# xdspacelab/openvslam

Hardware: NVIDIA H100
Metric: frames/sec extract+match+local-BA @1920x960 4000kp (higher is better)
Workload: dtype u8 (extract, Hamming) + f64 (pose optimiser, local BA)

## Files before the change

openvslam_b200/csrc/optimize.cu:

```cuda
#include <algorithm>
#include <cfloat>
#include <cmath>
#include <cstdio>
#include <cstdlib>
#include <cstring>
#include <new>
#include <sched.h>
#include <time.h>
#include <vector>


#include "ba_math.cuh"
#include "ovs_common.h"

namespace {

using ovs::CameraD;

constexpr int kMaxReducedDimBig = 6000;
constexpr int kCholMaxDynSmem = 226 * 1024;
constexpr int kNB = 32;
constexpr int kCholThreads = 512;
constexpr int kCholCluster = 8;
constexpr int kPoseThreads = 256;
// ... 62 lines not shown
    int stopped;
    int spec_width;
    int round_live;
    int need_more;
    int pending_nbatch;
    int num_rounds, num_iterations, num_trials, batches, solver_trials;
    int round_iterations[8];
    double lambda_init[8];
    double last_chi2, last_lambda;
};

struct BaDev {
    CameraD cam;
    int K, L, M, nfree, n;
    const double* poses; const double* points;
    const double* poses_ring; const double* points_ring;
    const int* obs_kf; const int* obs_lm; const float2* obs_xy; const float* obs_xr; const float* inv_sigma_sq;
    const unsigned char* level;
    const int* free_idx;
    const int* lm_first;
    int use_huber; double delta;
};

__global__ void __launch_bounds__(128) k_ba_linearize(BaDev P, const LmCtl* __restrict__ ctl, double* __restrict__ Hpl, double* __restrict__ Cpp,
                                                       double* __restrict__ bpo, double* __restrict__ All, double* __restrict__ blo) {
    if (!ctl->active) return;
    __shared__ __align__(16) double sm[128 * 30];
    P.poses = P.poses_ring + (size_t)ctl->cur * 12 * P.K; P.points = P.points_ring + (size_t)ctl->cur * 3 * P.L;
    P.use_huber = ctl->use_huber;
    const int base = blockIdx.x * 128, t = threadIdx.x;
    const int i = base + t;
    const int nedge = min(128, P.M - base);
    const bool live = i < P.M && !P.level[i];
    int dim = 0, fi = -1;
    double e[3] = {0, 0, 0}, Jp[18], Jl[9], ww = 0;
#pragma unroll
    for (int k = 0; k < 18; ++k) Jp[k] = 0;
#pragma unroll
    for (int k = 0; k < 9; ++k) Jl[k] = 0;
    if (live) {
        const int kf = P.obs_kf[i], lm = P.obs_lm[i];
        fi = P.free_idx[kf];
        const float xr = P.obs_xr ? P.obs_xr[i] : -1.0f;
        const bool stereo = xr >= 0.0f;
        const float2 xy = P.obs_xy[i];
        const double obs[3] = {(double)xy.x, (double)xy.y, (double)xr};
        double pose[12], pw[3];
#pragma unroll
        for (int k = 0; k < 12; ++k) pose[k] = P.poses[12 * (size_t)kf + k];
#pragma unroll
        for (int k = 0; k < 3; ++k) pw[k] = P.points[3 * (size_t)lm + k];
        dim = ovs::edge_eval(P.cam, pose, pw, obs, stereo, e, Jp, Jl);
        const double w = (double)P.inv_sigma_sq[i];
        double chi = 0;
        for (int d = 0; d < dim; ++d) chi += w * e[d] * e[d];
        double rho0 = chi, rho1 = 1.0;
        if (P.use_huber) ovs::huber(chi, P.delta, &rho0, &rho1);
        ww = rho1 * w;
    }
    double* sW = sm; double* sbp = sm + 128 * 18; double* sA = sbp + 128 * 6;
    {
        double* A = sA + 6 * t;
        for (int a = 0; a < 3; ++a)
            for (int b = a; b < 3; ++b) {
                double h = 0;
                for (int d = 0; d < dim; ++d) h += Jl[3 * d + a] * ww * Jl[3 * d + b];
                A[ovs::sym3(a, b)] = h;
            }
        double* W = sW + 18 * t; double* bp = sbp + 6 * t;
        const bool fr = fi >= 0;
        for (int a = 0; a < 6; ++a) {
            double g = 0;
            for (int d = 0; d < dim; ++d) g -= Jp[6 * d + a] * ww * e[d];
            bp[a] = fr ? g : 0.0;
            for (int b = 0; b < 3; ++b) {
                double h = 0;
                for (int d = 0; d < dim; ++d) h += Jp[6 * d + a] * ww * Jl[3 * d + b];
                W[3 * a + b] = fr ? h : 0.0;
            }
        }
    }
    __syncthreads();
    {
        const double2* s2 = reinterpret_cast<const double2*>(sW); double2* g2 = reinterpret_cast<double2*>(Hpl + 18 * (size_t)base);
        for (int q = t; q < 9 * nedge; q += 128) g2[q] = s2[q];
        s2 = reinterpret_cast<const double2*>(sbp); g2 = reinterpret_cast<double2*>(bpo + 6 * (size_t)base);
        for (int q = t; q < 3 * nedge; q += 128) g2[q] = s2[q];
        s2 = reinterpret_cast<const double2*>(sA); g2 = reinterpret_cast<double2*>(All + 6 * (size_t)base);
        for (int q = t; q < 3 * nedge; q += 128) g2[q] = s2[q];
    }
    __syncthreads();
    double* sC = sm; double* sbl = sm + 128 * 21;
    {
        double* C = sC + 21 * t; double* bl = sbl + 3 * t;
        const bool fr = fi >= 0;
        for (int a = 0; a < 6; ++a)
            for (int b = a; b < 6; ++b) {
                double h = 0;
                for (int d = 0; d < dim; ++d) h += Jp[6 * d + a] * ww * Jp[6 * d + b];
                C[ovs::sym6(a, b)] = fr ? h : 0.0;
            }
        for (int a = 0; a < 3; ++a) {
            double g = 0;
            for (int d = 0; d < dim; ++d) g -= Jl[3 * d + a] * ww * e[d];
            bl[a] = g;
        }
    }
    __syncthreads();
    {
        const double2* s2 = reinterpret_cast<const double2*>(sC); double2* g2 = reinterpret_cast<double2*>(Cpp + 21 * (size_t)base);
        const int nd = 21 * nedge;
        for (int q = t; q < nd / 2; q += 128) g2[q] = s2[q];
        if ((nd & 1) && t == 0) Cpp[21 * (size_t)base + nd - 1] = sC[nd - 1];
        const int nb = 3 * nedge;
        for (int q = t; q < nb; q += 128) blo[3 * (size_t)base + q] = sbl[q];
    }
}

__global__ void __launch_bounds__(128) k_ba_landmark_accum(BaDev P, const LmCtl* __restrict__ ctl, const double* __restrict__ All, const double* __restrict__ blo,
                                                            double* __restrict__ Hll, double* __restrict__ bl, double* __restrict__ maxdiag) {
    if (!ctl->active) return;
    const int l = blockIdx.x * 128 + threadIdx.x;
    double md = 0;
    if (l < P.L) {
        double H[6] = {0, 0, 0, 0, 0, 0}, b[3] = {0, 0, 0};
        for (int p = P.lm_first[l]; p < P.lm_first[l + 1]; ++p) {
            if (P.level[p]) continue;
#pragma unroll
            for (int k = 0; k < 6; ++k) H[k] += All[6 * (size_t)p + k];
#pragma unroll
            for (int k = 0; k < 3; ++k) b[k] += blo[3 * (size_t)p + k];
        }
#pragma unroll
        for (int k = 0; k < 6; ++k) Hll[6 * (size_t)l + k] = H[k];
#pragma unroll
        for (int k = 0; k < 3; ++k) bl[3 * (size_t)l + k] = b[k];
        md = fmax(fabs(H[0]), fmax(fabs(H[3]), fabs(H[5])));
    }
#pragma unroll
    for (int o = 16; o > 0; o >>= 1) md = fmax(md, __shfl_xor_sync(0xffffffffu, md, o));
    if ((threadIdx.x & 31) == 0 && md > 0) atomic_max_pos(maxdiag, md);
}

__global__ void __launch_bounds__(128) k_ba_pose_accum_chunk(BaDev P, const LmCtl* __restrict__ ctl, const int* __restrict__ nchunks,
                                                              const int4* __restrict__ pair_rec, const int4* __restrict__ chunks,
                                                              const double* __restrict__ Cpp, const double* __restrict__ bpo,
                                                              double* __restrict__ ppart) {
    __shared__ double red[27][4];
    if (!ctl->active || (int)blockIdx.x >= *nchunks) return;
    const int4 ch = chunks[blockIdx.x];
    const int e = ch.y + threadIdx.x;
    double acc[27];
#pragma unroll
    for (int k = 0; k < 27; ++k) acc[k] = 0;
    if (e < ch.z) {
        const int4 rec = pair_rec[e];
        const int o = rec.x;
        if (!rec.w) {
#pragma unroll
            for (int k = 0; k < 21; ++k) acc[k] = Cpp[21 * (size_t)o + k];
#pragma unroll
            for (int k = 0; k < 6; ++k) acc[21 + k] = bpo[6 * (size_t)o + k];
        }
    }
    const int lane = threadIdx.x & 31, wid = threadIdx.x >> 5;
#pragma unroll
    for (int k = 0; k < 27; ++k) {
        const double v = warp_sum(acc[k]);
        if (lane == 0) red[k][wid] = v;
    }
    __syncthreads();
    if (threadIdx.x < 27)
        ppart[27 * (size_t)blockIdx.x + threadIdx.x] = red[threadIdx.x][0] + red[threadIdx.x][1] + red[threadIdx.x][2] + red[threadIdx.x][3];
}

__global__ void k_ba_pose_final_plan(LmCtl* ctl, int nfree, const int* __restrict__ kf_chunk_begin, const double* __restrict__ ppart,
                                     double* __restrict__ Hpp, double* __restrict__ bp, double* maxdiag, int* fail,
                                     const volatile int* stop_word, volatile int* mirror);

__device__ __forceinline__ void dmma_m8n8k4(double& d0, double& d1, double a, double b) {
    asm volatile("mma.sync.aligned.m8n8k4.row.col.f64.f64.f64.f64 {%0, %1}, {%2}, {%3}, {%0, %1};\n" : "+d"(d0), "+d"(d1) : "d"(a), "d"(b));
}

constexpr int kSGY = 76, kSGW = 84;
__global__ void __launch_bounds__(128, 4) k_ba_schur_chunk(BaDev P, const LmCtl* __restrict__ ctl, const int* __restrict__ nchunks,
                                                         const int4* __restrict__ pair_rec, const int4* __restrict__ chunks,
                                                         const int2* __restrict__ pair_ab, const double* __restrict__ Hll,
                                                         const double* __restrict__ Hpl, const double* __restrict__ bl,
                                                         double* __restrict__ spart, size_t spart_stride) {
    __shared__ double s_y[4 * 8 * kSGY];
    __shared__ double s_w[4 * 8 * kSGW];
    double* sYw = s_y + (threadIdx.x >> 5) * 8 * kSGY;
    double* sWw = s_w + (threadIdx.x >> 5) * 8 * kSGW;
    static_assert(4 * 8 * kSGY >= kSpec * 4 * 64, "reduction buffer must fit in the Y region");
    const int nbatch = ctl->nbatch;
    if (nbatch == 0 || (int)blockIdx.x >= *nchunks) return;
// ... 757 lines not shown
                ovs::pose_oplus(pose, u, out);
            } else {
#pragma unroll
                for (int j = 0; j < 12; ++j) out[j] = pose[j];
            }
            double* cand_poses = poses_ring + (size_t)buf[bt] * 12 * P.K;
#pragma unroll
            for (int j = 0; j < 12; ++j) cand_poses[12 * (size_t)k + j] = out[j];
            }
        }
    }
#pragma unroll
    for (int bt = 0; bt < kSpec; ++bt) {
        if (bt < nbatch) {
            const double tot = block_sum(sc[bt], sm);
            if (threadIdx.x == 0) partial_scale[(size_t)bt * gridDim.x + blockIdx.x] = tot;
        }
    }
}

__global__ void __launch_bounds__(128) k_ba_errors(BaDev P, const LmCtl* __restrict__ ctl, int at_current,
                                                    double* __restrict__ err, double* __restrict__ partial_chi) {
    __shared__ double sm[36];
    int slot;
    if (at_current) {
        if (!ctl->active) return;
        slot = ctl->cur;
    } else {
        if ((int)blockIdx.y >= ctl->nbatch) return;
        slot = ctl->buf[blockIdx.y];
    }
    P.use_huber = ctl->use_huber;
    P.poses = P.poses_ring + (size_t)slot * 12 * P.K;
    P.points = P.points_ring + (size_t)slot * 3 * P.L;
    err += (size_t)blockIdx.y * 3 * P.M; partial_chi += (size_t)blockIdx.y * gridDim.x;
    const int i = blockIdx.x * 128 + threadIdx.x;
    double c = 0;
    if (i < P.M && !P.level[i]) {
        const int kf = P.obs_kf[i];
        const float xr = P.obs_xr ? P.obs_xr[i] : -1.0f;
        const bool stereo = xr >= 0.0f;
        const float2 xy = P.obs_xy[i];
        const double obs[3] = {(double)xy.x, (double)xy.y, (double)xr};
        double pose[12], pw[3], e[3] = {0, 0, 0};
#pragma unroll
        for (int k = 0; k < 12; ++k) pose[k] = P.poses[12 * (size_t)kf + k];
        const size_t pi = P.obs_lm ? (size_t)P.obs_lm[i] : (size_t)i;
#pragma unroll
        for (int k = 0; k < 3; ++k) pw[k] = P.points[3 * pi + k];
        ovs::edge_eval(P.cam, pose, pw, obs, stereo, e, nullptr, nullptr);
        err[3 * (size_t)i] = e[0]; err[3 * (size_t)i + 1] = e[1]; err[3 * (size_t)i + 2] = stereo ? e[2] : 0.0;
        const double w = (double)P.inv_sigma_sq[i];
        double chi = w * (e[0] * e[0] + e[1] * e[1]);
        if (stereo) chi += w * e[2] * e[2];
        c = chi;
        if (P.use_huber) { double r1; ovs::huber(chi, P.delta, &c, &r1); }
    }
    const double tot = block_sum(c, sm);
    if (threadIdx.x == 0) partial_chi[blockIdx.x] = tot;
}

__device__ __forceinline__ void mirror_state(const LmCtl& c, volatile int* mirror) {
    if (!mirror) return;
    mirror[0] = c.nbatch; mirror[1] = c.active; mirror[3] = c.need_more; mirror[4] = c.it;
}

__global__ void __launch_bounds__(kSpec * 256) k_ba_reduce(LmCtl* ctl, int mode, const double* __restrict__ partial_chi, int nchi,
                                                           const double* __restrict__ partial_scale, int nscale, int* fail,
                                                           const volatile int* stop_word, int batch_index, int* exec_log, volatile int* mirror,
                                                           int halt_if_undecided, int next_width_cap) {
    __shared__ double sm[kSpec][2][8];
    const int nb = mode == 0 ? (ctl->active ? 1 : 0) : ctl->nbatch;
    if (nb == 0) {
        if (threadIdx.x == 0 && mode == 1 && exec_log && batch_index >= 0) exec_log[batch_index] = 0;
        return;
    }
    const int t = threadIdx.x >> 8, tl = threadIdx.x & 255, lane = tl & 31, w = tl >> 5;
    double a = 0, b = 0;
    if (t < nb) {
        const double* pc = partial_chi + (size_t)t * nchi;
        for (int i = tl; i < nchi; i += 256) a += pc[i];
        if (mode == 1) {
// ... 488 lines not shown
            int ws = wsum[lane];
#pragma unroll
            for (int o = 1; o < 32; o <<= 1) { const int u = __shfl_up_sync(0xffffffffu, ws, o); if (lane >= o) ws += u; }
            wsum[lane] = ws;
        }
        __syncthreads();
        const int excl = carry + (wid ? wsum[wid - 1] : 0) + v - c;
        if (i < count) chunk_begin[i] = excl;
        __syncthreads();
        if (tid == 1023) carry = excl + c;
        __syncthreads();
    }
    if (tid == 0) { chunk_begin[count] = carry; *total = carry; }
}

__global__ void __launch_bounds__(128) k_ba_chunk_fill(const int* __restrict__ ids, int count, const int* __restrict__ seg_begin,
                                                        const int* __restrict__ seg_end, const int* __restrict__ chunk_begin, int4* __restrict__ chunks) {
    const int i = blockIdx.x * 128 + threadIdx.x;
    if (i >= count) return;
    const int id = ids ? ids[i] : i;
    const int e1 = seg_end[id];
    int c = chunk_begin[i];
    for (int e0 = seg_begin[id]; e0 < e1; e0 += 128, ++c) chunks[c] = make_int4(i, e0, min(e0 + 128, e1), 0);
}

struct PoseOptArgs {
    CameraD cam;
    int n;
    const double* pts_w; const float2* obs_xy; const float* obs_xr; const float* inv_sigma_sq;
    double* pose;
    unsigned char* outlier;
    int num_trials, num_each_iter;
    double delta, chi2_2d, chi2_3d;
    double* stats;
};

__device__ bool solve6(const double* Hs , double lambda, const double* b, double* x) {
    double Lm[6][6];
    for (int i = 0; i < 6; ++i)
        for (int j = 0; j <= i; ++j) {
            double s = Hs[ovs::sym6(j, i)] + (i == j ? lambda : 0.0);
            for (int k = 0; k < j; ++k) s -= Lm[i][k] * Lm[j][k];
            if (i == j) {
                if (!(s > 0.0) || !isfinite(s)) return false;
                Lm[i][i] = sqrt(s);
            } else Lm[i][j] = s / Lm[j][j];
// ... 212 lines not shown
        const double e0 = err[3 * (size_t)i], e1 = err[3 * (size_t)i + 1], e2 = err[3 * (size_t)i + 2];
        fc[0] += w * (e0 * e0 + e1 * e1) + (stereo ? w * e2 * e2 : 0.0);
    }
    reduce_all(fc, 1);
    if (gtid == 0) {
        A.stats[0] = total_iters; A.stats[1] = total_trials; A.stats[2] = rounds; A.stats[3] = s_sys[0]; A.stats[4] = n - num_bad;
    }
    if (gtid < 12) A.pose[gtid] = s_pose[gtid];
}

}

struct ovs_ba_plan;
extern "C" void ovs_optimizer_destroy(ovs_optimizer* h);
struct ovs_optimizer {
    int device = 0;
    ovs_ba_plan* plan = nullptr;
    cudaStream_t stream = nullptr;
    cudaEvent_t ev[2]{};
    std::vector<cudaEvent_t> solver_ev;
    cudaGraphExec_t gx_iter = nullptr;
    int spec_width = kSpec;
    int spec_width2 = 0;
    int use_graphs = 0;
    int lm_host_sync = -1;
    bool pending = false;
    uint8_t* d_arena = nullptr; size_t d_cap = 0;
    uint8_t* h_arena = nullptr; size_t h_cap = 0;
    uint8_t* d_work = nullptr; size_t w_cap = 0;
    int* h_mirror = nullptr;
    int* d_mirror = nullptr;
    int chol_cluster = kCholCluster;
};

namespace {

struct Arena {
    uint8_t* base; size_t off, cap;
    template <typename T> T* take(size_t n) {
        off = (off + 255) / 256 * 256;
        T* p = reinterpret_cast<T*>(base + off);
        off += n * sizeof(T);
        return p;
    }
};

int ensure_arenas(ovs_optimizer* h, size_t dbytes, size_t hbytes) {
// ... 78 lines not shown
        stats->final_chi2 = hstats[3];
        for (int r = 0; r < 8 && r < stats->num_rounds; ++r) stats->lambda_init[r] = hstats[5 + r];
        float ms = 0; cudaEventElapsedTime(&ms, h->ev[0], h->ev[1]);
        stats->device_us = ms * 1000.f;
    }
    return OVS_OK;
}

struct ovs_ba_plan {
    bool valid = false;
    BaDev P{};
    int K = 0, L = 0, M = 0, nfree = 0, n = 0, npairs = 0, nb_obs = 0, nb_upd = 0;
    long long npair_entries = 0;
    size_t chol_smem = 0;
    int chol_dbuf = 0, chol_big = 0;
    double* hposes = nullptr; double* hpoints = nullptr; uint8_t* hout = nullptr;
    LmCtl* hctl = nullptr; int* hexec = nullptr; int exec_cap = 0;
    double *dposes_in = nullptr, *dpoints_in = nullptr;
    double *dposes_ring = nullptr, *dpoints_ring = nullptr;
    uint8_t* dlevel = nullptr; double* derr = nullptr;
    uint8_t* dout = nullptr;
    LmCtl* dctl = nullptr; int* dexec = nullptr;
    size_t spart_stride = 0, S_stride = 0, invL_stride = 0;
    double *dHpl = nullptr, *dCpp = nullptr, *dbpo = nullptr, *dAll = nullptr, *dblo = nullptr;
    double *dHll = nullptr, *dbl = nullptr, *dHpp = nullptr, *dbp = nullptr;
    double *dS = nullptr, *dbS = nullptr, *dx = nullptr, *dinvL = nullptr;
    int4* d_pair_rec = nullptr; int *dsegb = nullptr, *dsege = nullptr; int2* dpab = nullptr; int* ddiag = nullptr;
    int4 *dchunks = nullptr, *ddchunks = nullptr; int *dpair_chunk_begin = nullptr, *dkf_chunk_begin = nullptr;
    int* dnchunks = nullptr;
    double *dspart = nullptr, *dppart = nullptr; int max_chunks = 0, max_dchunks = 0;
    double *dpchi = nullptr, *dpscale = nullptr; int* dfail = nullptr; double* dmaxdiag = nullptr; long long* dclk = nullptr;
    int cur = 0;
};

namespace {

struct BaInputs {
    const double* poses; const uint8_t* fixed; const double* points; const int32_t* obs_kf; const int32_t* obs_lm;
    const float* obs_xy; const float* obs_x_right; const float* inv_sigma_sq;
};

int ensure_work(ovs_optimizer* h, size_t bytes) {
    if (bytes > h->w_cap) {
        cudaFree(h->d_work); h->d_work = nullptr; h->w_cap = 0;
        bytes += bytes / 4;
        OVS_CUDA_CHECK(cudaMalloc(&h->d_work, bytes));
        h->w_cap = bytes;
    }
    return OVS_OK;
}

int prepare_impl(ovs_optimizer* h, const ovs_camera* cam, int setup_is_mono, int K, int L, int M, const BaInputs& in, bool on_device) {
    OVS_REQUIRE(h && cam && K > 0 && L > 0 && M > 0, OVS_ERR_INVALID_ARG, "bad argument");
// ... 5 lines not shown
    cudaStream_t st = h->stream;
    if (h->pending) { OVS_CUDA_CHECK(ovs::sync_stream(st)); h->pending = false; }

    const size_t sM = (size_t)M, sL = (size_t)L, sK = (size_t)K;
    const int nb_obs = (M + 127) / 128, nb_upd = (L + K + 127) / 128;
    const int exec_cap = 1024;
    double* hposes; double* hpoints; int *hkf, *hlm; float *hxy, *hxr, *hw; uint8_t* hfixed; uint8_t* hout; long long* hcounts;
    double* dposes_in; double* dpoints_in; int *dkf, *dlm; float *dxy, *dxr, *dw; uint8_t* dfixed;
    int *dfree, *dlmf, *dpoff; long long* dcounts;
    size_t in_bytes = 0;
    auto carve1 = [&](Arena& H, Arena& D) {
        hposes = H.take<double>(12 * sK); hpoints = H.take<double>(3 * sL);
        hkf = H.take<int>(sM); hlm = H.take<int>(sM); hxy = H.take<float>(2 * sM); hxr = H.take<float>(sM); hw = H.take<float>(sM);
        hfixed = H.take<uint8_t>(sK);
        in_bytes = H.off;
        hout = H.take<uint8_t>(sM); pl.hctl = H.take<LmCtl>(1); pl.hexec = H.take<int>(exec_cap); hcounts = H.take<long long>(8);
        dposes_in = D.take<double>(12 * sK); dpoints_in = D.take<double>(3 * sL);
        dkf = D.take<int>(sM); dlm = D.take<int>(sM); dxy = D.take<float>(2 * sM); dxr = D.take<float>(sM); dw = D.take<float>(sM);
        dfixed = D.take<uint8_t>(sK);
        dfree = D.take<int>(sK); dlmf = D.take<int>(sL + 1); dpoff = D.take<int>(sL + 1); dcounts = D.take<long long>(8);
        pl.dout = D.take<uint8_t>(sM); pl.dctl = D.take<LmCtl>(1); pl.dexec = D.take<int>(exec_cap);
        pl.dposes_ring = D.take<double>((kSpec + 1) * 12 * sK); pl.dpoints_ring = D.take<double>((kSpec + 1) * 3 * sL);
        pl.dlevel = D.take<uint8_t>(sM); pl.derr = D.take<double>(kSpec * 3 * sM);
        pl.dHpl = D.take<double>(18 * sM); pl.dCpp = D.take<double>(21 * sM); pl.dbpo = D.take<double>(6 * sM);
        pl.dAll = D.take<double>(6 * sM); pl.dblo = D.take<double>(3 * sM);
        pl.dHll = D.take<double>(6 * sL); pl.dbl = D.take<double>(3 * sL);
        pl.dpchi = D.take<double>(kSpec * (size_t)nb_obs); pl.dpscale = D.take<double>(kSpec * (size_t)nb_upd);
        pl.dfail = D.take<int>(kSpec); pl.dmaxdiag = D.take<double>(2); pl.dclk = D.take<long long>(192); pl.dnchunks = D.take<int>(2);
    };
    {
        Arena H0{nullptr, 0, 0}, D0{nullptr, 0, 0};
        carve1(H0, D0);
        const int rc = ensure_arenas(h, D0.off + 256, H0.off + 256);
        if (rc != OVS_OK) return rc;
    }
    Arena H{h->h_arena, 0, h->h_cap}, D{h->d_arena, 0, h->d_cap};
    carve1(H, D);
    pl.exec_cap = exec_cap;
    h->pending = true;
    if (!on_device) {
        memcpy(hposes, in.poses, 96 * sK); memcpy(hpoints, in.points, 24 * sL);
        memcpy(hkf, in.obs_kf, 4 * sM); memcpy(hlm, in.obs_lm, 4 * sM); memcpy(hxy, in.obs_xy, 8 * sM); memcpy(hw, in.inv_sigma_sq, 4 * sM);
        if (in.obs_x_right) memcpy(hxr, in.obs_x_right, 4 * sM); else for (size_t i = 0; i < sM; ++i) hxr[i] = -1.0f;
        memcpy(hfixed, in.fixed, sK);
        OVS_CUDA_CHECK(cudaMemcpyAsync(h->d_arena, h->h_arena, in_bytes, cudaMemcpyHostToDevice, st));
    } else {
        const cudaMemcpyKind dd = cudaMemcpyDeviceToDevice;
// ... 16 lines not shown
    OVS_LAUNCH_CHECK();
    OVS_CUDA_CHECK(cudaMemcpyAsync(hcounts, dcounts, 5 * sizeof(long long), cudaMemcpyDeviceToHost, st));
    OVS_CUDA_CHECK(ovs::sync_stream(st));
    if (hcounts[4] != 0x7fffffffffffffffll) {
        const long long i = hcounts[4] >> 2;
        const int code = (int)(hcounts[4] & 3);
        h->pending = false;
        if (code == 2) { ovs::set_error("observations must be grouped by landmark (obs_lm non-decreasing; first violation at observation %lld)", i); return OVS_ERR_INVALID_ARG; }
        if (!on_device) ovs::set_error("observation %lld references keyframe %d / landmark %d out of range", i, in.obs_kf[i], in.obs_lm[i]);
        else ovs::set_error("observation %lld references a keyframe / landmark out of range", i);
        return OVS_ERR_INVALID_ARG;
    }
    const int nfree = (int)hcounts[0];
    const long long npair_entries = hcounts[1], nfree_edges = hcounts[2];
    const int n = 6 * nfree;
    OVS_REQUIRE(nfree >= 1, OVS_ERR_INVALID_ARG, "no free keyframe");
    OVS_REQUIRE(n <= kMaxReducedDimBig, OVS_ERR_UNSUPPORTED, "more than %d free keyframes", kMaxReducedDimBig / 6);
    OVS_REQUIRE(npair_entries < (1ll << 30), OVS_ERR_UNSUPPORTED, "too many co-observations");
    const int npairs = nfree * (nfree + 1) / 2;

    const size_t sE = (size_t)std::max<long long>(npair_entries, 1);
    const size_t max_chunks = sE / 128 + (size_t)npairs + 8;
    const size_t max_dchunks = (size_t)nfree_edges / 128 + (size_t)nfree + 8;
    unsigned *dkeys, *dkeys2; unsigned long long *dvals, *dvals2; int4* dprec; int* dsort;
    auto carve2 = [&](Arena& W) {
        pl.dpab = W.take<int2>(npairs); pl.ddiag = W.take<int>(nfree);
        pl.dHpp = W.take<double>(21 * (size_t)nfree); pl.dbp = W.take<double>(6 * (size_t)nfree);
        pl.S_stride = ((size_t)(n + 1) * n + 31) / 32 * 32; pl.invL_stride = (size_t)((n + kNB - 1) / kNB) * kNB * kNB;
        pl.dS = W.take<double>(kSpec * pl.S_stride); pl.dbS = pl.dS + (size_t)n * n; pl.dx = W.take<double>(kSpec * (size_t)n);
        pl.dinvL = W.take<double>(kSpec * pl.invL_stride);
        dkeys = W.take<unsigned>(sE); dkeys2 = W.take<unsigned>(sE);
        dvals = W.take<unsigned long long>(sE); dvals2 = W.take<unsigned long long>(sE); dprec = W.take<int4>(sE);
        dsort = W.take<int>(sort_scratch_ints((long long)sE));
        pl.dsegb = W.take<int>(npairs); pl.dsege = W.take<int>(npairs);
        pl.dchunks = W.take<int4>(max_chunks); pl.ddchunks = W.take<int4>(max_dchunks);
        pl.dpair_chunk_begin = W.take<int>(npairs + 1); pl.dkf_chunk_begin = W.take<int>(nfree + 1);
        pl.spart_stride = 42 * max_chunks;
        pl.dspart = W.take<double>(kSpec * pl.spart_stride); pl.dppart = W.take<double>(27 * max_dchunks);
    };
    {
        Arena W0{nullptr, 0, 0};
        carve2(W0);
        const int rc = ensure_work(h, W0.off + 256);
        if (rc != OVS_OK) return rc;
    }
    Arena W{h->d_work, 0, h->w_cap};
    carve2(W);
    pl.max_chunks = (int)max_chunks; pl.max_dchunks = (int)max_dchunks;
    OVS_CUDA_CHECK(cudaMemsetAsync(pl.dsegb, 0, 4 * (size_t)npairs, st));
    OVS_CUDA_CHECK(cudaMemsetAsync(pl.dsege, 0, 4 * (size_t)npairs, st));
    OVS_CUDA_CHECK(cudaMemsetAsync(pl.dS, 0, 8 * kSpec * pl.S_stride, st));

    BaDev& P = pl.P;
    P.cam = to_cam(cam); P.K = K; P.L = L; P.M = M; P.nfree = nfree; P.n = n;
    P.poses = dposes_in; P.points = dpoints_in; P.poses_ring = pl.dposes_ring; P.points_ring = pl.dpoints_ring;
    P.obs_kf = dkf; P.obs_lm = dlm; P.obs_xy = (const float2*)dxy; P.obs_xr = dxr; P.inv_sigma_sq = dw;
    P.level = pl.dlevel; P.free_idx = dfree; P.lm_first = dlmf;
    const float chi_sq_2D = 5.99146f, chi_sq_3D = 7.81473f;
    P.use_huber = 1; P.delta = (double)(setup_is_mono ? sqrtf(chi_sq_2D) : sqrtf(chi_sq_3D));

    k_ba_pair_table<<<nfree, 128, 0, st>>>(nfree, pl.dpab, pl.ddiag);
    OVS_LAUNCH_CHECK();
    pl.d_pair_rec = dprec;
    if (npair_entries > 0) {
        k_ba_emit_pairs<<<(L + 127) / 128, 128, 0, st>>>(P, dpoff, dkeys, dvals);
        OVS_LAUNCH_CHECK();
        int end_bit = 1;
        while ((1 << end_bit) < npairs) ++end_bit;
        unsigned* ksorted = nullptr; unsigned long long* vsorted = nullptr;
        const int src = sort_pairs(st, dkeys, dkeys2, dvals, dvals2, (int)npair_entries, end_bit, dsort, &ksorted, &vsorted);
        if (src != OVS_OK) return src;
        k_ba_segments<<<((int)npair_entries + 255) / 256, 256, 0, st>>>(ksorted, (int)npair_entries, pl.dsegb, pl.dsege);
        OVS_LAUNCH_CHECK();
        k_ba_pair_records<<<((int)npair_entries + 255) / 256, 256, 0, st>>>(vsorted, (int)npair_entries, dlm, dprec);
        OVS_LAUNCH_CHECK();
    }
    k_ba_chunk_scan<<<1, 1024, 0, st>>>(nullptr, npairs, pl.dsegb, pl.dsege, pl.dpair_chunk_begin, pl.dnchunks);
    OVS_LAUNCH_CHECK();
    k_ba_chunk_fill<<<(npairs + 127) / 128, 128, 0, st>>>(nullptr, npairs, pl.dsegb, pl.dsege, pl.dpair_chunk_begin, pl.dchunks);
    OVS_LAUNCH_CHECK();
    k_ba_chunk_scan<<<1, 1024, 0, st>>>(pl.ddiag, nfree, pl.dsegb, pl.dsege, pl.dkf_chunk_begin, pl.dnchunks + 1);
    OVS_LAUNCH_CHECK();
    k_ba_chunk_fill<<<(nfree + 127) / 128, 128, 0, st>>>(pl.ddiag, nfree, pl.dsegb, pl.dsege, pl.dkf_chunk_begin, pl.ddchunks);
    OVS_LAUNCH_CHECK();

    pl.K = K; pl.L = L; pl.M = M; pl.nfree = nfree; pl.n = n; pl.npairs = npairs; pl.nb_obs = nb_obs; pl.nb_upd = nb_upd;
    pl.npair_entries = npair_entries;
    {
        const size_t fixed = chol_fixed_doubles(n), panel = chol_panel_doubles(n), back = chol_back_doubles(n) - 32 * 33;
        const size_t one = (fixed + std::max(panel, back)) * sizeof(double);
        const size_t two = (fixed + std::max(panel, back + chol_back_doubles(n))) * sizeof(double);
        pl.chol_big = one > (size_t)kCholMaxDynSmem ? 1 : 0;
        pl.chol_dbuf = two <= (size_t)kCholMaxDynSmem ? 1 : 0;
        pl.chol_smem = pl.chol_big ? 0 : (pl.chol_dbuf ? two : one);
    }
    pl.hposes = hposes; pl.hpoints = hpoints; pl.hout = hout;
    pl.dposes_in = dposes_in; pl.dpoints_in = dpoints_in;
    pl.cur = 0;
    pl.valid = true;
    return OVS_OK;
}

}

extern "C" int ovs_local_ba_prepare(ovs_optimizer* h, const ovs_camera* cam, int setup_is_mono, int K, const double* poses,
                                    const uint8_t* fixed, int L, const double* points, int M, const int32_t* obs_kf,
                                    const int32_t* obs_lm, const float* obs_xy, const float* obs_x_right, const float* inv_sigma_sq) {
// ... 118 lines not shown
            OVS_CUDA_CHECK(cudaLaunchKernelEx(&cfg, k_ba_cholesky_solve, (const LmCtl*)ctl, pl.dS, pl.S_stride, n, pl.dx, pl.dinvL, pl.invL_stride, pl.dfail, pl.dclk, pl.chol_dbuf));
            ovs::count_launch();
        } else {
            for (int kb = 0; kb < n; kb += kNB) {
                const int nb = std::min(kNB, n - kb), rem = n - kb - nb, prow = rem + 1;
                k_chol_big_diag<<<dim3(1, kSpec), 64, 0, st>>>(ctl, pl.dS, pl.S_stride, n, kb, nb, pl.dinvL, pl.invL_stride, pl.dfail);
                OVS_LAUNCH_CHECK();
                k_chol_big_panel<<<dim3((prow + 127) / 128, kSpec), 128, 0, st>>>(ctl, pl.dS, pl.S_stride, n, kb, nb, pl.dinvL, pl.invL_stride);
                OVS_LAUNCH_CHECK();
                if (rem > 0) {
                    int tiles = 0;
                    for (int mi = 0; mi < (prow + 15) / 16; ++mi) tiles += std::min((rem + 31) / 32, (16 * mi + 15) / 32 + 1);
                    k_chol_big_trailing<<<dim3((tiles + 3) / 4, kSpec), 128, 0, st>>>(ctl, pl.dS, pl.S_stride, n, kb, nb);
                    OVS_LAUNCH_CHECK();
                }
            }
            const size_t bsm = (size_t)(((n + 31) / 32) * 32 + 32 * 33 + 32) * sizeof(double);
            k_chol_big_backsolve<<<kSpec, 512, bsm, st>>>(ctl, pl.dS, pl.S_stride, n, pl.dinvL, pl.invL_stride, pl.dx, pl.dfail);
            OVS_LAUNCH_CHECK();
        }
        if (ev) OVS_CUDA_CHECK(cudaEventRecord(h->solver_ev[4 * slot + 3], st));
        k_ba_update<<<nb_upd, 128, 0, st>>>(P, ctl, pl.dHpl, pl.dHll, pl.dbl, pl.dbp, pl.dx, pl.dposes_ring, pl.dpoints_ring, pl.dpscale, pl.dfail);
        OVS_LAUNCH_CHECK();
        k_ba_errors<<<dim3(nb_obs, kSpec), 128, 0, st>>>(P, ctl, 0, pl.derr, pl.dpchi);
        OVS_LAUNCH_CHECK();
        k_ba_reduce<<<1, kSpec * 256, 0, st>>>(ctl, 1, pl.dpchi, nb_obs, pl.dpscale, nb_upd, pl.dfail, stop_word, ev ? slot : -1, pl.dexec, mirror,
                                               halt_if_undecided ? 1 : 0, next_width_cap);
        OVS_LAUNCH_CHECK();
        if (!in_graph) ++solver_slots;
        return OVS_OK;
    };

    auto iteration_head = [&](bool in_graph, bool halt_if_undecided) -> int {
        k_ba_linearize<<<nb_obs, 128, 0, st>>>(P, ctl, pl.dHpl, pl.dCpp, pl.dbpo, pl.dAll, pl.dblo);
        OVS_LAUNCH_CHECK();
        k_ba_landmark_accum<<<(L + 127) / 128, 128, 0, st>>>(P, ctl, pl.dAll, pl.dblo, pl.dHll, pl.dbl, pl.dmaxdiag);
        OVS_LAUNCH_CHECK();
        k_ba_pose_accum_chunk<<<pl.max_dchunks, 128, 0, st>>>(P, ctl, pl.dnchunks + 1, pl.d_pair_rec, pl.ddchunks, pl.dCpp, pl.dbpo, pl.dppart);
        OVS_LAUNCH_CHECK();
        k_ba_pose_final_plan<<<1, 1024, 0, st>>>(ctl, nfree, pl.dkf_chunk_begin, pl.dppart, pl.dHpp, pl.dbp, pl.dmaxdiag, pl.dfail, stop_word, mirror);
        OVS_LAUNCH_CHECK();
        if (sw2 > 0 && halt_if_undecided) {
            const int rc = trial_batch(in_graph, false, sw2);
            if (rc != OVS_OK) return rc;
        }
        return trial_batch(in_graph, halt_if_undecided, 0);
    };

    auto finish_iteration = [&]() -> int {
        for (;;) {
            int rc = wait_device();
            if (rc != OVS_OK) return rc;
            if (hm[0] == 0) return OVS_OK;
            rc = trial_batch(false, false, 0);
            if (rc != OVS_OK) return rc;
        }
    };

    auto lm_optimize = [&](int iterations, int use_huber) -> int {
        k_lm_round_begin<<<1, 1, 0, st>>>(ctl, iterations, use_huber, stop_word, pl.dmaxdiag, mirror);
        OVS_LAUNCH_CHECK();
// ... 115 lines not shown
    return run_impl(h, 2, 1, num_first_iter, num_second_iter, force_stop_flag, stats);
}

extern "C" int ovs_global_ba_host(ovs_optimizer* h, const ovs_camera* cam, int setup_is_mono, int K, double* poses, const uint8_t* fixed,
                                  int L, double* points, int M, const int32_t* obs_kf, const int32_t* obs_lm, const float* obs_xy,
                                  const float* obs_x_right, const float* inv_sigma_sq, int num_iter, int use_huber_kernel,
                                  const volatile uint8_t* force_stop_flag, ovs_ba_stats* stats) {
    OVS_REQUIRE(h && cam && K > 0 && L >= 0 && M >= 0 && num_iter >= 0, OVS_ERR_INVALID_ARG, "bad argument");
    OVS_REQUIRE(poses && fixed && (L == 0 || points) && (M == 0 || (obs_kf && obs_lm && obs_xy && inv_sigma_sq)), OVS_ERR_INVALID_ARG, "null argument");
    if (stats) memset(stats, 0, sizeof(*stats));
    if (force_stop_flag && *force_stop_flag) return OVS_OK;
    if (M == 0 || L == 0) return OVS_OK;
    int rc = ovs_local_ba_prepare(h, cam, setup_is_mono, K, poses, fixed, L, points, M, obs_kf, obs_lm, obs_xy, obs_x_right, inv_sigma_sq);
    if (rc != OVS_OK) return rc;
    rc = run_impl(h, 1, use_huber_kernel ? 1 : 0, num_iter, 0, force_stop_flag, stats);
    if (rc != OVS_OK) return rc;
    return ovs_local_ba_fetch(h, poses, points, nullptr);
}

extern "C" int ovs_optimizer_cluster_width(const ovs_optimizer* h) { return h ? h->chol_cluster : 0; }

extern "C" int ovs_optimizer_set_cluster_width(ovs_optimizer* h, int width) {
    OVS_REQUIRE(h && (width == 1 || width == 2 || width == 4 || width == 8), OVS_ERR_INVALID_ARG, "cluster width must be 1, 2, 4 or 8");
    h->chol_cluster = width;
    return OVS_OK;
}

extern "C" int ovs_optimizer_set_speculation(ovs_optimizer* h, int width) {
    OVS_REQUIRE(h && width >= 1 && width <= kSpec, OVS_ERR_INVALID_ARG, "speculation width must be 1..%d", kSpec);
    h->spec_width = width;
    return OVS_OK;
}

extern "C" int ovs_optimizer_set_second_batch(ovs_optimizer* h, int width) {
    OVS_REQUIRE(h && width >= 0 && width <= kSpec, OVS_ERR_INVALID_ARG, "second-batch width must be 0..%d", kSpec);
    h->spec_width2 = width;
    return OVS_OK;
}

extern "C" int ovs_optimizer_set_graphs(ovs_optimizer* h, int enable) {
    OVS_REQUIRE(h, OVS_ERR_INVALID_ARG, "null handle");
    h->use_graphs = enable ? 1 : 0;
    return OVS_OK;
}

extern "C" int ovs_optimizer_set_host_sync(ovs_optimizer* h, int mode) {
// ... 138 lines not shown
```

Measured before the change: 387.1.

## Fuse pose accumulation into linearize, batch speculative error eval, enable graphs

Result: faster. 397.3, median of 6 (+2.6%).

```diff
diff --git a/openvslam_b200/csrc/optimize.cu b/openvslam_b200/csrc/optimize.cu
--- a/openvslam_b200/csrc/optimize.cu
+++ b/openvslam_b200/csrc/optimize.cu
@@ -108,99 +108,127 @@
     int use_huber; double delta;
 };
 
-__global__ void __launch_bounds__(128) k_ba_linearize(BaDev P, const LmCtl* __restrict__ ctl, double* __restrict__ Hpl, double* __restrict__ Cpp,
-                                                       double* __restrict__ bpo, double* __restrict__ All, double* __restrict__ blo) {
+__device__ __forceinline__ int ba_edge_linearize(const BaDev& P, int i, int lm, const double* pose, double* e, double* Jp, double* Jl, double& ww) {
+    const float xr = P.obs_xr ? P.obs_xr[i] : -1.0f;
+    const bool stereo = xr >= 0.0f;
+    const float2 xy = P.obs_xy[i];
+    const double obs[3] = {(double)xy.x, (double)xy.y, (double)xr};
+    double pw[3];
+#pragma unroll
+    for (int k = 0; k < 3; ++k) pw[k] = P.points[3 * (size_t)lm + k];
+    const int dim = ovs::edge_eval(P.cam, pose, pw, obs, stereo, e, Jp, Jl);
+    const double w = (double)P.inv_sigma_sq[i];
+    double chi = 0;
+    for (int d = 0; d < dim; ++d) chi += w * e[d] * e[d];
+    double rho0 = chi, rho1 = 1.0;
+    if (P.use_huber) ovs::huber(chi, P.delta, &rho0, &rho1);
+    ww = rho1 * w;
+    return dim;
+}
+__device__ __forceinline__ void ba_store_landmark_blocks(int i, int dim, const double* e, const double* Jl, double ww,
+                                                         double* __restrict__ All, double* __restrict__ blo) {
+    double A[6];
+#pragma unroll
+    for (int a = 0; a < 3; ++a)
+#pragma unroll
+        for (int b = a; b < 3; ++b) {
+            double h = 0;
+            for (int d = 0; d < dim; ++d) h += Jl[3 * d + a] * ww * Jl[3 * d + b];
+            A[ovs::sym3(a, b)] = h;
+        }
+    double2* A2 = reinterpret_cast<double2*>(All + 6 * (size_t)i);
+#pragma unroll
+    for (int k = 0; k < 3; ++k) A2[k] = make_double2(A[2 * k], A[2 * k + 1]);
+#pragma unroll
+    for (int a = 0; a < 3; ++a) {
+        double g = 0;
+        for (int d = 0; d < dim; ++d) g -= Jl[3 * d + a] * ww * e[d];
+        blo[3 * (size_t)i + a] = g;
+    }
+}
+
+__global__ void __launch_bounds__(128) k_ba_linearize(BaDev P, const LmCtl* __restrict__ ctl, const int* __restrict__ nchunks,
+                                                       const int4* __restrict__ pair_rec, const int4* __restrict__ chunks, int dchunk_cap,
+                                                       const int* __restrict__ fixed_edges, int nfixed, double* __restrict__ Hpl,
+                                                       double* __restrict__ All, double* __restrict__ blo, double* __restrict__ ppart) {
+    __shared__ double spose[12];
+    __shared__ double red[27][4];
     if (!ctl->active) return;
-    __shared__ __align__(16) double sm[128 * 30];
     P.poses = P.poses_ring + (size_t)ctl->cur * 12 * P.K; P.points = P.points_ring + (size_t)ctl->cur * 3 * P.L;
     P.use_huber = ctl->use_huber;
-    const int base = blockIdx.x * 128, t = threadIdx.x;
-    const int i = base + t;
-    const int nedge = min(128, P.M - base);
-    const bool live = i < P.M && !P.level[i];
-    int dim = 0, fi = -1;
+    const int t = threadIdx.x;
+    int dim = 0;
     double e[3] = {0, 0, 0}, Jp[18], Jl[9], ww = 0;
 #pragma unroll
     for (int k = 0; k < 18; ++k) Jp[k] = 0;
 #pragma unroll
     for (int k = 0; k < 9; ++k) Jl[k] = 0;
+    if ((int)blockIdx.x >= dchunk_cap) {
+        const int j = ((int)blockIdx.x - dchunk_cap) * 128 + t;
+        if (j >= nfixed) return;
+        const int i = fixed_edges[j];
+        if (!P.level[i]) {
+            const int kf = P.obs_kf[i];
+            double pose[12];
+#pragma unroll
+            for (int k = 0; k < 12; ++k) pose[k] = P.poses[12 * (size_t)kf + k];
+            dim = ba_edge_linearize(P, i, P.obs_lm[i], pose, e, Jp, Jl, ww);
+        }
+        ba_store_landmark_blocks(i, dim, e, Jl, ww, All, blo);
+        return;
+    }
+    if ((int)blockIdx.x >= *nchunks) return;
+    const int4 ch = chunks[blockIdx.x];
+    if (t < 12) spose[t] = P.poses[12 * (size_t)P.obs_kf[pair_rec[ch.y].x] + t];
+    const int r = ch.y + t;
+    const bool has = r < ch.z;
+    int4 rec = make_int4(0, 0, 0, 1);
+    if (has) rec = pair_rec[r];
+    const int i = rec.x;
+    const bool live = has && !P.level[i];
+    __syncthreads();
     if (live) {
-        const int kf = P.obs_kf[i], lm = P.obs_lm[i];
-        fi = P.free_idx[kf];
-        const float xr = P.obs_xr ? P.obs_xr[i] : -1.0f;
-        const bool stereo = xr >= 0.0f;
-        const float2 xy = P.obs_xy[i];
-        const double obs[3] = {(double)xy.x, (double)xy.y, (double)xr};
-        double pose[12], pw[3];
-#pragma unroll
-        for (int k = 0; k < 12; ++k) pose[k] = P.poses[12 * (size_t)kf + k];
-#pragma unroll
-        for (int k = 0; k < 3; ++k) pw[k] = P.points[3 * (size_t)lm + k];
-        dim = ovs::edge_eval(P.cam, pose, pw, obs, stereo, e, Jp, Jl);
-        const double w = (double)P.inv_sigma_sq[i];
-        double chi = 0;
-        for (int d = 0; d < dim; ++d) chi += w * e[d] * e[d];
-        double rho0 = chi, rho1 = 1.0;
-        if (P.use_huber) ovs::huber(chi, P.delta, &rho0, &rho1);
-        ww = rho1 * w;
-    }
-    double* sW = sm; double* sbp = sm + 128 * 18; double* sA = sbp + 128 * 6;
-    {
-        double* A = sA + 6 * t;
-        for (int a = 0; a < 3; ++a)
-            for (int b = a; b < 3; ++b) {
-                double h = 0;
-                for (int d = 0; d < dim; ++d) h += Jl[3 * d + a] * ww * Jl[3 * d + b];
-                A[ovs::sym3(a, b)] = h;
-            }
-        double* W = sW + 18 * t; double* bp = sbp + 6 * t;
-        const bool fr = fi >= 0;
-        for (int a = 0; a < 6; ++a) {
-            double g = 0;
-            for (int d = 0; d < dim; ++d) g -= Jp[6 * d + a] * ww * e[d];
-            bp[a] = fr ? g : 0.0;
+        double pose[12];
+#pragma unroll
+        for (int k = 0; k < 12; ++k) pose[k] = spose[k];
+        dim = ba_edge_linearize(P, i, rec.z, pose, e, Jp, Jl, ww);
+    }
+    if (has) {
+        double W[18];
+#pragma unroll
+        for (int a = 0; a < 6; ++a)
+#pragma unroll
             for (int b = 0; b < 3; ++b) {
                 double h = 0;
                 for (int d = 0; d < dim; ++d) h += Jp[6 * d + a] * ww * Jl[3 * d + b];
-                W[3 * a + b] = fr ? h : 0.0;
-            }
-        }
+                W[3 * a + b] = h;
+            }
+        double2* W2 = reinterpret_cast<double2*>(Hpl + 18 * (size_t)i);
+#pragma unroll
+        for (int k = 0; k < 9; ++k) W2[k] = make_double2(W[2 * k], W[2 * k + 1]);
+        ba_store_landmark_blocks(i, dim, e, Jl, ww, All, blo);
+    }
+    const bool add = has && !rec.w;
+    const int lane = t & 31, wid = t >> 5;
+#pragma unroll
+    for (int a = 0; a < 6; ++a)
+#pragma unroll
+        for (int b = a; b < 6; ++b) {
+            double h = 0;
+            for (int d = 0; d < dim; ++d) h += Jp[6 * d + a] * ww * Jp[6 * d + b];
+            const double v = warp_sum(add ? h : 0.0);
+            if (lane == 0) red[ovs::sym6(a, b)][wid] = v;
+        }
+#pragma unroll
+    for (int a = 0; a < 6; ++a) {
+        double g = 0;
+        for (int d = 0; d < dim; ++d) g -= Jp[6 * d + a] * ww * e[d];
+        const double v = warp_sum(add ? g : 0.0);
+        if (lane == 0) red[21 + a][wid] = v;
     }
     __syncthreads();
-    {
-        const double2* s2 = reinterpret_cast<const double2*>(sW); double2* g2 = reinterpret_cast<double2*>(Hpl + 18 * (size_t)base);
-        for (int q = t; q < 9 * nedge; q += 128) g2[q] = s2[q];
-        s2 = reinterpret_cast<const double2*>(sbp); g2 = reinterpret_cast<double2*>(bpo + 6 * (size_t)base);
-        for (int q = t; q < 3 * nedge; q += 128) g2[q] = s2[q];
-        s2 = reinterpret_cast<const double2*>(sA); g2 = reinterpret_cast<double2*>(All + 6 * (size_t)base);
-        for (int q = t; q < 3 * nedge; q += 128) g2[q] = s2[q];
-    }
-    __syncthreads();
-    double* sC = sm; double* sbl = sm + 128 * 21;
-    {
-        double* C = sC + 21 * t; double* bl = sbl + 3 * t;
-        const bool fr = fi >= 0;
-        for (int a = 0; a < 6; ++a)
-            for (int b = a; b < 6; ++b) {
-                double h = 0;
-                for (int d = 0; d < dim; ++d) h += Jp[6 * d + a] * ww * Jp[6 * d + b];
-                C[ovs::sym6(a, b)] = fr ? h : 0.0;
-            }
-        for (int a = 0; a < 3; ++a) {
-            double g = 0;
-            for (int d = 0; d < dim; ++d) g -= Jl[3 * d + a] * ww * e[d];
-            bl[a] = g;
-        }
-    }
-    __syncthreads();
-    {
-        const double2* s2 = reinterpret_cast<const double2*>(sC); double2* g2 = reinterpret_cast<double2*>(Cpp + 21 * (size_t)base);
-        const int nd = 21 * nedge;
-        for (int q = t; q < nd / 2; q += 128) g2[q] = s2[q];
-        if ((nd & 1) && t == 0) Cpp[21 * (size_t)base + nd - 1] = sC[nd - 1];
-        const int nb = 3 * nedge;
-        for (int q = t; q < nb; q += 128) blo[3 * (size_t)base + q] = sbl[q];
-    }
+    if (t < 27)
+        ppart[27 * (size_t)blockIdx.x + t] = red[t][0] + red[t][1] + red[t][2] + red[t][3];
 }
 
 __global__ void __launch_bounds__(128) k_ba_landmark_accum(BaDev P, const LmCtl* __restrict__ ctl, const double* __restrict__ All, const double* __restrict__ blo,
@@ -226,38 +254,6 @@
 #pragma unroll
     for (int o = 16; o > 0; o >>= 1) md = fmax(md, __shfl_xor_sync(0xffffffffu, md, o));
     if ((threadIdx.x & 31) == 0 && md > 0) atomic_max_pos(maxdiag, md);
-}
-
-__global__ void __launch_bounds__(128) k_ba_pose_accum_chunk(BaDev P, const LmCtl* __restrict__ ctl, const int* __restrict__ nchunks,
-                                                              const int4* __restrict__ pair_rec, const int4* __restrict__ chunks,
-                                                              const double* __restrict__ Cpp, const double* __restrict__ bpo,
-                                                              double* __restrict__ ppart) {
-    __shared__ double red[27][4];
-    if (!ctl->active || (int)blockIdx.x >= *nchunks) return;
-    const int4 ch = chunks[blockIdx.x];
-    const int e = ch.y + threadIdx.x;
-    double acc[27];
-#pragma unroll
-    for (int k = 0; k < 27; ++k) acc[k] = 0;
-    if (e < ch.z) {
-        const int4 rec = pair_rec[e];
-        const int o = rec.x;
-        if (!rec.w) {
-#pragma unroll
-            for (int k = 0; k < 21; ++k) acc[k] = Cpp[21 * (size_t)o + k];
-#pragma unroll
-            for (int k = 0; k < 6; ++k) acc[21 + k] = bpo[6 * (size_t)o + k];
-        }
-    }
-    const int lane = threadIdx.x & 31, wid = threadIdx.x >> 5;
-#pragma unroll
-    for (int k = 0; k < 27; ++k) {
-        const double v = warp_sum(acc[k]);
-        if (lane == 0) red[k][wid] = v;
-    }
-    __syncthreads();
-    if (threadIdx.x < 27)
-        ppart[27 * (size_t)blockIdx.x + threadIdx.x] = red[threadIdx.x][0] + red[threadIdx.x][1] + red[threadIdx.x][2] + red[threadIdx.x][3];
 }
 
 __global__ void k_ba_pose_final_plan(LmCtl* ctl, int nfree, const int* __restrict__ kf_chunk_begin, const double* __restrict__ ppart,
@@ -1061,42 +1057,56 @@
 __global__ void __launch_bounds__(128) k_ba_errors(BaDev P, const LmCtl* __restrict__ ctl, int at_current,
                                                     double* __restrict__ err, double* __restrict__ partial_chi) {
     __shared__ double sm[36];
-    int slot;
+    int nb, slot[kSpec];
     if (at_current) {
         if (!ctl->active) return;
-        slot = ctl->cur;
+        nb = 1; slot[0] = ctl->cur;
     } else {
-        if ((int)blockIdx.y >= ctl->nbatch) return;
-        slot = ctl->buf[blockIdx.y];
+        nb = ctl->nbatch;
+        if (nb == 0) return;
+#pragma unroll
+        for (int bt = 0; bt < kSpec; ++bt) slot[bt] = ctl->buf[bt];
     }
     P.use_huber = ctl->use_huber;
-    P.poses = P.poses_ring + (size_t)slot * 12 * P.K;
-    P.points = P.points_ring + (size_t)slot * 3 * P.L;
-    err += (size_t)blockIdx.y * 3 * P.M; partial_chi += (size_t)blockIdx.y * gridDim.x;
     const int i = blockIdx.x * 128 + threadIdx.x;
-    double c = 0;
+    double c[kSpec];
+#pragma unroll
+    for (int bt = 0; bt < kSpec; ++bt) c[bt] = 0;
     if (i < P.M && !P.level[i]) {
         const int kf = P.obs_kf[i];
         const float xr = P.obs_xr ? P.obs_xr[i] : -1.0f;
         const bool stereo = xr >= 0.0f;
         const float2 xy = P.obs_xy[i];
         const double obs[3] = {(double)xy.x, (double)xy.y, (double)xr};
-        double pose[12], pw[3], e[3] = {0, 0, 0};
-#pragma unroll
-        for (int k = 0; k < 12; ++k) pose[k] = P.poses[12 * (size_t)kf + k];
         const size_t pi = P.obs_lm ? (size_t)P.obs_lm[i] : (size_t)i;
-#pragma unroll
-        for (int k = 0; k < 3; ++k) pw[k] = P.points[3 * pi + k];
-        ovs::edge_eval(P.cam, pose, pw, obs, stereo, e, nullptr, nullptr);
-        err[3 * (size_t)i] = e[0]; err[3 * (size_t)i + 1] = e[1]; err[3 * (size_t)i + 2] = stereo ? e[2] : 0.0;
         const double w = (double)P.inv_sigma_sq[i];
-        double chi = w * (e[0] * e[0] + e[1] * e[1]);
-        if (stereo) chi += w * e[2] * e[2];
-        c = chi;
-        if (P.use_huber) { double r1; ovs::huber(chi, P.delta, &c, &r1); }
-    }
-    const double tot = block_sum(c, sm);
-    if (threadIdx.x == 0) partial_chi[blockIdx.x] = tot;
+#pragma unroll
+        for (int bt = 0; bt < kSpec; ++bt) {
+            if (bt < nb) {
+                const double* poses = P.poses_ring + (size_t)slot[bt] * 12 * P.K;
+                const double* points = P.points_ring + (size_t)slot[bt] * 3 * P.L;
+                double pose[12], pw[3], e[3] = {0, 0, 0};
+#pragma unroll
+                for (int k = 0; k < 12; ++k) pose[k] = poses[12 * (size_t)kf + k];
+#pragma unroll
+                for (int k = 0; k < 3; ++k) pw[k] = points[3 * pi + k];
+                ovs::edge_eval(P.cam, pose, pw, obs, stereo, e, nullptr, nullptr);
+                double* eb = err + (size_t)bt * 3 * P.M;
+                eb[3 * (size_t)i] = e[0]; eb[3 * (size_t)i + 1] = e[1]; eb[3 * (size_t)i + 2] = stereo ? e[2] : 0.0;
+                double chi = w * (e[0] * e[0] + e[1] * e[1]);
+                if (stereo) chi += w * e[2] * e[2];
+                c[bt] = chi;
+                if (P.use_huber) { double r1; ovs::huber(chi, P.delta, &c[bt], &r1); }
+            }
+        }
+    }
+#pragma unroll
+    for (int bt = 0; bt < kSpec; ++bt) {
+        if (bt < nb) {
+            const double tot = block_sum(c[bt], sm);
+            if (threadIdx.x == 0) partial_chi[(size_t)bt * gridDim.x + blockIdx.x] = tot;
+        }
+    }
 }
 
 __device__ __forceinline__ void mirror_state(const LmCtl& c, volatile int* mirror) {
@@ -1631,6 +1641,30 @@
     const int e1 = seg_end[id];
     int c = chunk_begin[i];
     for (int e0 = seg_begin[id]; e0 < e1; e0 += 128, ++c) chunks[c] = make_int4(i, e0, min(e0 + 128, e1), 0);
+}
+
+__global__ void __launch_bounds__(1024) k_ba_fixed_count(int M, const int* __restrict__ obs_kf, const int* __restrict__ free_idx,
+                                                          int* __restrict__ tile_count) {
+    const int i = blockIdx.x * 1024 + threadIdx.x;
+    const int c = __syncthreads_count(i < M && free_idx[obs_kf[i]] < 0);
+    if (threadIdx.x == 0) tile_count[blockIdx.x] = c;
+}
+__global__ void __launch_bounds__(1024) k_ba_fixed_list(int M, const int* __restrict__ obs_kf, const int* __restrict__ free_idx,
+                                                         const int* __restrict__ tile_count, int* __restrict__ list) {
+    __shared__ int wsum[32], wcnt[32];
+    const int tid = threadIdx.x, lane = tid & 31, wid = tid >> 5;
+    int s = 0;
+    for (int b = tid; b < (int)blockIdx.x; b += 1024) s += tile_count[b];
+    s = __reduce_add_sync(0xffffffffu, s);
+    const int i = blockIdx.x * 1024 + tid;
+    const bool f = i < M && free_idx[obs_kf[i]] < 0;
+    const unsigned m = __ballot_sync(0xffffffffu, f);
+    if (lane == 0) { wsum[wid] = s; wcnt[wid] = __popc(m); }
+    __syncthreads();
+    if (!f) return;
+    int off = 0;
+    for (int w = 0; w < 32; ++w) off += wsum[w] + (w < wid ? wcnt[w] : 0);
+    list[off + __popc(m & ((1u << lane) - 1u))] = i;
 }
 
 struct PoseOptArgs {
@@ -1889,7 +1923,7 @@
     cudaGraphExec_t gx_iter = nullptr;
     int spec_width = kSpec;
     int spec_width2 = 0;
-    int use_graphs = 0;
+    int use_graphs = 1;
     int lm_host_sync = -1;
     bool pending = false;
     uint8_t* d_arena = nullptr; size_t d_cap = 0;
@@ -2014,13 +2048,14 @@
     uint8_t* dout = nullptr;
     LmCtl* dctl = nullptr; int* dexec = nullptr;
     size_t spart_stride = 0, S_stride = 0, invL_stride = 0;
-    double *dHpl = nullptr, *dCpp = nullptr, *dbpo = nullptr, *dAll = nullptr, *dblo = nullptr;
+    double *dHpl = nullptr, *dAll = nullptr, *dblo = nullptr;
     double *dHll = nullptr, *dbl = nullptr, *dHpp = nullptr, *dbp = nullptr;
     double *dS = nullptr, *dbS = nullptr, *dx = nullptr, *dinvL = nullptr;
     int4* d_pair_rec = nullptr; int *dsegb = nullptr, *dsege = nullptr; int2* dpab = nullptr; int* ddiag = nullptr;
     int4 *dchunks = nullptr, *ddchunks = nullptr; int *dpair_chunk_begin = nullptr, *dkf_chunk_begin = nullptr;
     int* dnchunks = nullptr;
     double *dspart = nullptr, *dppart = nullptr; int max_chunks = 0, max_dchunks = 0;
+    int* dfixed_edges = nullptr; int nfixed = 0;
     double *dpchi = nullptr, *dpscale = nullptr; int* dfail = nullptr; double* dmaxdiag = nullptr; long long* dclk = nullptr;
     int cur = 0;
 };
@@ -2072,7 +2107,7 @@
         pl.dout = D.take<uint8_t>(sM); pl.dctl = D.take<LmCtl>(1); pl.dexec = D.take<int>(exec_cap);
         pl.dposes_ring = D.take<double>((kSpec + 1) * 12 * sK); pl.dpoints_ring = D.take<double>((kSpec + 1) * 3 * sL);
         pl.dlevel = D.take<uint8_t>(sM); pl.derr = D.take<double>(kSpec * 3 * sM);
-        pl.dHpl = D.take<double>(18 * sM); pl.dCpp = D.take<double>(21 * sM); pl.dbpo = D.take<double>(6 * sM);
+        pl.dHpl = D.take<double>(18 * sM);
         pl.dAll = D.take<double>(6 * sM); pl.dblo = D.take<double>(3 * sM);
         pl.dHll = D.take<double>(6 * sL); pl.dbl = D.take<double>(3 * sL);
         pl.dpchi = D.take<double>(kSpec * (size_t)nb_obs); pl.dpscale = D.take<double>(kSpec * (size_t)nb_upd);
@@ -2135,6 +2170,8 @@
     const size_t sE = (size_t)std::max<long long>(npair_entries, 1);
     const size_t max_chunks = sE / 128 + (size_t)npairs + 8;
     const size_t max_dchunks = (size_t)nfree_edges / 128 + (size_t)nfree + 8;
+    const int nfixed = (int)(M - nfree_edges), nb_fix = (M + 1023) / 1024;
+    int* dfix_count;
     unsigned *dkeys, *dkeys2; unsigned long long *dvals, *dvals2; int4* dprec; int* dsort;
     auto carve2 = [&](Arena& W) {
         pl.dpab = W.take<int2>(npairs); pl.ddiag = W.take<int>(nfree);
@@ -2150,6 +2187,7 @@
         pl.dpair_chunk_begin = W.take<int>(npairs + 1); pl.dkf_chunk_begin = W.take<int>(nfree + 1);
         pl.spart_stride = 42 * max_chunks;
         pl.dspart = W.take<double>(kSpec * pl.spart_stride); pl.dppart = W.take<double>(27 * max_dchunks);
+        pl.dfixed_edges = W.take<int>(std::max(nfixed, 1)); dfix_count = W.take<int>(nb_fix);
     };
     {
         Arena W0{nullptr, 0, 0};
@@ -2159,7 +2197,7 @@
     }
     Arena W{h->d_work, 0, h->w_cap};
     carve2(W);
-    pl.max_chunks = (int)max_chunks; pl.max_dchunks = (int)max_dchunks;
+    pl.max_chunks = (int)max_chunks; pl.max_dchunks = (int)max_dchunks; pl.nfixed = nfixed;
     OVS_CUDA_CHECK(cudaMemsetAsync(pl.dsegb, 0, 4 * (size_t)npairs, st));
     OVS_CUDA_CHECK(cudaMemsetAsync(pl.dsege, 0, 4 * (size_t)npairs, st));
     OVS_CUDA_CHECK(cudaMemsetAsync(pl.dS, 0, 8 * kSpec * pl.S_stride, st));
@@ -2196,6 +2234,12 @@
     OVS_LAUNCH_CHECK();
     k_ba_chunk_fill<<<(nfree + 127) / 128, 128, 0, st>>>(pl.ddiag, nfree, pl.dsegb, pl.dsege, pl.dkf_chunk_begin, pl.ddchunks);
     OVS_LAUNCH_CHECK();
+    if (nfixed > 0) {
+        k_ba_fixed_count<<<nb_fix, 1024, 0, st>>>(M, dkf, dfree, dfix_count);
+        OVS_LAUNCH_CHECK();
+        k_ba_fixed_list<<<nb_fix, 1024, 0, st>>>(M, dkf, dfree, dfix_count, pl.dfixed_edges);
+        OVS_LAUNCH_CHECK();
+    }
 
     pl.K = K; pl.L = L; pl.M = M; pl.nfree = nfree; pl.n = n; pl.npairs = npairs; pl.nb_obs = nb_obs; pl.nb_upd = nb_upd;
     pl.npair_entries = npair_entries;
@@ -2360,7 +2404,7 @@
         if (ev) OVS_CUDA_CHECK(cudaEventRecord(h->solver_ev[4 * slot + 3], st));
         k_ba_update<<<nb_upd, 128, 0, st>>>(P, ctl, pl.dHpl, pl.dHll, pl.dbl, pl.dbp, pl.dx, pl.dposes_ring, pl.dpoints_ring, pl.dpscale, pl.dfail);
         OVS_LAUNCH_CHECK();
-        k_ba_errors<<<dim3(nb_obs, kSpec), 128, 0, st>>>(P, ctl, 0, pl.derr, pl.dpchi);
+        k_ba_errors<<<nb_obs, 128, 0, st>>>(P, ctl, 0, pl.derr, pl.dpchi);
         OVS_LAUNCH_CHECK();
         k_ba_reduce<<<1, kSpec * 256, 0, st>>>(ctl, 1, pl.dpchi, nb_obs, pl.dpscale, nb_upd, pl.dfail, stop_word, ev ? slot : -1, pl.dexec, mirror,
                                                halt_if_undecided ? 1 : 0, next_width_cap);
@@ -2370,11 +2414,10 @@
     };
 
     auto iteration_head = [&](bool in_graph, bool halt_if_undecided) -> int {
-        k_ba_linearize<<<nb_obs, 128, 0, st>>>(P, ctl, pl.dHpl, pl.dCpp, pl.dbpo, pl.dAll, pl.dblo);
+        k_ba_linearize<<<pl.max_dchunks + (pl.nfixed + 127) / 128, 128, 0, st>>>(P, ctl, pl.dnchunks + 1, pl.d_pair_rec, pl.ddchunks, pl.max_dchunks,
+                                                                                pl.dfixed_edges, pl.nfixed, pl.dHpl, pl.dAll, pl.dblo, pl.dppart);
         OVS_LAUNCH_CHECK();
         k_ba_landmark_accum<<<(L + 127) / 128, 128, 0, st>>>(P, ctl, pl.dAll, pl.dblo, pl.dHll, pl.dbl, pl.dmaxdiag);
-        OVS_LAUNCH_CHECK();
-        k_ba_pose_accum_chunk<<<pl.max_dchunks, 128, 0, st>>>(P, ctl, pl.dnchunks + 1, pl.d_pair_rec, pl.ddchunks, pl.dCpp, pl.dbpo, pl.dppart);
         OVS_LAUNCH_CHECK();
         k_ba_pose_final_plan<<<1, 1024, 0, st>>>(ctl, nfree, pl.dkf_chunk_begin, pl.dppart, pl.dHpp, pl.dbp, pl.dmaxdiag, pl.dfail, stop_word, mirror);
         OVS_LAUNCH_CHECK();
@@ -2536,6 +2579,12 @@
 
 extern "C" int ovs_optimizer_set_cluster_width(ovs_optimizer* h, int width) {
     OVS_REQUIRE(h && (width == 1 || width == 2 || width == 4 || width == 8), OVS_ERR_INVALID_ARG, "cluster width must be 1, 2, 4 or 8");
+    if (width != h->chol_cluster && h->gx_iter) {
+        OVS_CUDA_CHECK(cudaSetDevice(h->device));
+        OVS_CUDA_CHECK(ovs::sync_stream(h->stream));
+        cudaGraphExecDestroy(h->gx_iter);
+        h->gx_iter = nullptr;
+    }
     h->chol_cluster = width;
     return OVS_OK;
 }
```
